# leopard-ai/betty

Hardware: AMD Instinct MI355X
Metric: hypergradient-steps/sec (CG K=20, 10M inner params) (higher is better)
Workload: dtype f32

## Files before the change

betty_amd/csrc/bhg_common.hpp:

```cpp
#pragma once
#include <hip/hip_runtime.h>
#include <stdint.h>
#include <stddef.h>
#include <stdio.h>
#include <string.h>

#include "bhg.h"

namespace bhg {

constexpr int kThreads = 256;
constexpr int kWaves = kThreads / 64;
constexpr int kChunk = BHG_CHUNK_ELEMS;
constexpr int kVecPerThread = kChunk / (kThreads * 4);
constexpr int kMaxBlocks = 1024;
constexpr int kInlineT = 32;
constexpr int kWriterT = 448;

constexpr size_t kWsScal = 0;
constexpr size_t kWsPartP = 128;
constexpr size_t kWsPartR = kWsPartP + 8 * kMaxBlocks;
constexpr size_t kWsBarrier = kWsPartR + 16 * kMaxBlocks;
constexpr size_t kWsTables = kWsBarrier + 256;
inline size_t ws_bytes(int T) {
  size_t b = kWsTables + 4 * sizeof(void*) * (size_t)(T > 0 ? T : 0);
  return (b + 255) & ~(size_t)255;
}

enum { S_RR_OLD = 0, S_PHP = 1, S_ALPHA = 2, S_RR_NEW = 3, S_BETA = 4, S_PP = 5 , S_ALPHA_RING = 10 ,
       S_NPART0 = 8  };

#define BHG_DBG_KEYS(X)                                                                                                      \
  X(mlp_wsk) X(mlp_wsk_maxk) X(mlp_wsk_depth) X(mlp_wsk_lds) X(wsl_depth) X(no_nt_slabs) X(gemm_no_xpose) X(mlp_no_fast)      \
  X(mlp_tn) X(split_target) X(split_cap) X(mlp_no_head) X(gram_ksplit) X(gram_kchunk) X(proj_graw_split) X(mlp_proj)         \
  X(mlp_hoist) X(hoist_wgs) X(proj_step_alone) X(mlp_no_side) X(mlp_no_fuse) X(mlp_no_outer_all) X(neumann_side)             \
  X(hoist_staged_mink) X(proj_alpha_alone) X(proj_small_alone) X(outer_order_by_work) X(outer_no_pre) X(outer_stagger)       \
  X(mlp_no_fused_solve) X(cg_eager_p) X(cg_x_every_iter) X(neumann_p_every_iter) X(head_no_prefetch) X(cg_spin_limit)        \
  X(packed_chain) X(packed_depth) X(packed_gram) X(proj_max_ratio) X(proj_ws_cap_mb) X(alpha_in_hoist) X(graw_v2) X(wskp_ragged) X(pstep_v2) X(pstep_unroll) X(rnew_in_graw) X(graw_cols) X(lin_first) X(lin_prio) X(lin_nub) X(lin_order) X(lin_update_next) X(lin_withhold_beta) X(neumann_vnew) X(cg_rhs_direct) X(packed_prepare) X(lin_deep) X(graw_kloop) X(lin_update_in_head) X(xcd_pairs) X(headu_head_first) X(fx_ksplit) X(head_j) X(head_j_tile)
enum DbgKey : int {
#define BHG_DBG_ENUM(n) DBG_##n,
  BHG_DBG_KEYS(BHG_DBG_ENUM)
#undef BHG_DBG_ENUM
  DBG_COUNT
};
constexpr int kDbgUnset = INT32_MIN;
#ifdef BHG_AB
extern int g_dbg[DBG_COUNT];
inline bool dbg_is_set(DbgKey k) { return g_dbg[k] != kDbgUnset; }
inline int dbg(DbgKey k, int dflt) { return g_dbg[k] == kDbgUnset ? dflt : g_dbg[k]; }
#else
constexpr bool dbg_is_set(DbgKey) { return false; }
constexpr int dbg(DbgKey, int dflt) { return dflt; }
#endif

constexpr int kStampKernels = 4, kStampBlocks = 4096, kStampSlots = 8;
#ifdef BHG_STAMPS
#ifdef __HIPCC__
#define BHG_STAMP(kid, slot)                                                                                            \
  do {                                                                                                                  \
    if (threadIdx.x == 0 && blockIdx.x < ::bhg::kStampBlocks) {                                                         \
      unsigned long long* sp_ = ::bhg::d_stamps;                                                                        \
      if (sp_) sp_[((kid) * ::bhg::kStampBlocks + blockIdx.x) * ::bhg::kStampSlots + (slot)] = wall_clock64();          \
    }                                                                                                                   \
  } while (0)
#endif
#else
#define BHG_STAMP(kid, slot) do { } while (0)
#endif

void set_error(const char* fmt, ...);
#define BHG_HIP_CHECK(expr)                                                        \
  do {                                                                             \
    hipError_t _e = (expr);                                                        \
    if (_e != hipSuccess) {                                                        \
      ::bhg::set_error("%s failed: %s (%s:%d)", #expr, hipGetErrorString(_e), __FILE__, \
                       __LINE__);                                                  \
      return BHG_ERR_HIP;                                                          \
    }                                                                              \
  } while (0)
#define BHG_REQUIRE(cond, msg)                                                     \
  do {                                                                             \
    if (!(cond)) {                                                                 \
      ::bhg::set_error("%s: %s", __func__, msg);                                   \
      return BHG_ERR_ARG;                                                          \
    }                                                                              \
  } while (0)

struct PtrTab {
  const void* const* dev;
  const void* inl[kInlineT];
};

int make_table(PtrTab* out, const void* const* host_ptrs, int T, void* ws, int slot,
               hipStream_t stream);

bool span_begin(int kind, hipEvent_t* a, hipEvent_t* b);

#ifdef __HIPCC__
__device__ __forceinline__ float* tab_ptr(const PtrTab& t, int i) {
  const void* p = t.dev ? t.dev[i] : t.inl[i];
  return (float*)p;
}

__device__ __forceinline__ float4 ld4(const float* __restrict__ base, int e, int len) {
  if (e + 4 <= len) return *reinterpret_cast<const float4*>(base + e);
  float4 r = make_float4(0.f, 0.f, 0.f, 0.f);
  if (e < len) r.x = base[e];
  if (e + 1 < len) r.y = base[e + 1];
  if (e + 2 < len) r.z = base[e + 2];
  return r;
}
__device__ __forceinline__ void st4(float* __restrict__ base, int e, int len, float4 v) {
  if (e + 4 <= len) {
    *reinterpret_cast<float4*>(base + e) = v;
    return;
  }
  if (e < len) base[e] = v.x;
  if (e + 1 < len) base[e + 1] = v.y;
  if (e + 2 < len) base[e + 2] = v.z;
}

// ... 142 lines not shown
```

betty_amd/csrc/bhg_mlp.hip:

```cpp
#include <stdlib.h>


#include "bhg_common.hpp"
#include "bhg_mlp_headj.hpp"

#ifdef BHG_STAMPS
namespace bhg { __device__ unsigned long long* d_stamps = nullptr; }
#endif

namespace bhg {
namespace {
#include "mlp/gemm.inc"

#include "mlp/outer.inc"

#include "mlp/scalars.inc"

#include "mlp/head.inc"

#include "mlp/wsk.inc"

#include "mlp/wskp.inc"

inline int wsk_mode(int chain_mode, int unfused_hint) {
  if (dbg_is_set(DBG_mlp_wsk)) return dbg(DBG_mlp_wsk, 0);
  if (chain_mode == FUSE_CG) return 2;
  if (chain_mode == FUSE_NEUMANN) return 3;
  return unfused_hint;
}
inline bool wsk_wanted(int mode, int pairs, int K) {
  if (mode == 1) return true;
  if (mode != 2 && mode != 3) return false;
  return pairs * K <= dbg(DBG_mlp_wsk_maxk, 1024);
}
inline int wsk_depth() {
  const int d = dbg(DBG_mlp_wsk_depth, 3);
  return d == 2 ? 2 : 3;
}
inline bool wsk_eligible(const WskArgs& a) {
  if (a.pairs < 1 || a.pairs > 2) return false;
  bool ok = a.M % 32 == 0 && a.N % 32 == 0 && a.K % 32 == 0 && a.K >= 32;
  for (int i = 0; i < a.pairs; ++i) ok = ok && (a.pr[i].lda & 3) == 0 && (a.pr[i].ldb & 3) == 0;
  return ok;
}
int64_t g_wsk_launches = 0;
int64_t g_hoist_launches = 0;
int64_t g_proj_iterations = 0;
int64_t g_lin_launches = 0;
template <int LB>
void launch_gemm_wsk(const WskArgs& a_in, hipStream_t st, bool staged = false) {
  WskArgs a = a_in;
  ++g_wsk_launches;
  a.ntm = a.M / 32;
  a.ntn = a.N / 32;
  bool bf = false;
  for (int i = 0; i < a.pairs; ++i) bf = bf || a.pr[i].mix != 0;
  const dim3 grid(a.ntm * a.ntn), block(64 * kWskWaves);
  const int d = wsk_depth();
  const bool force_staged = dbg(DBG_mlp_wsk_lds, 0) != 0;
  if ((staged || force_staged) && !bf) {
    const int lds = (int)(sizeof(float) * kWslWaveFloats * kWskWaves);
    static bool attr_done = false;
    if (!attr_done) {
      (void)hipFuncSetAttribute(reinterpret_cast<const void*>(k_gemm_wsk<LB, false, 2, true>), hipFuncAttributeMaxDynamicSharedMemorySize, lds);
      attr_done = true;
    }
#ifdef BHG_AB
    const int wsl_depth = dbg(DBG_wsl_depth, 2);
    if (wsl_depth == 3) {
      static bool attr3 = false;
      if (!attr3) {
        (void)hipFuncSetAttribute(reinterpret_cast<const void*>(k_gemm_wsk<LB, false, 3, true>), hipFuncAttributeMaxDynamicSharedMemorySize, lds);
        attr3 = true;
      }
      hipLaunchKernelGGL((k_gemm_wsk<LB, false, 3, true>), grid, block, lds, st, a);
      return;
    }
#endif
    hipLaunchKernelGGL((k_gemm_wsk<LB, false, 2, true>), grid, block, lds, st, a);
    return;
  }
#define BHG_WSK(BFV, DV) hipLaunchKernelGGL((k_gemm_wsk<LB, BFV, DV>), grid, block, 0, st, a)
  if (bf) {
    if (d == 2 || LB == LAYOUT_RC) BHG_WSK(true, 2); else BHG_WSK(true, LB == LAYOUT_RC ? 2 : 3);
  } else {
#ifdef BHG_AB
    if (d == 2) BHG_WSK(false, 2); else
// ... 428 lines not shown
  memset(w, 0, sizeof(*w));
  const bool head = use_head(m);
  int nrr = bias_blocks(m);
  for (int l = 0; l < m->L; ++l) nrr += outer_blocks(m, l, head);
  w->nRR = nrr;
  size_t off = 0;
  auto take = [&](size_t bytes) { void* p = base ? static_cast<char*>(base) + off : nullptr; off += (bytes + 255) & ~(size_t)255; return p; };
  w->partT1 = static_cast<double*>(take(sizeof(double) * m->Bp));
  w->partT2h = static_cast<double*>(take(sizeof(double) * m->Bp));
  w->partPP = static_cast<double*>(take(sizeof(double) * kMaxBlocks));
  w->partRR[0] = static_cast<double*>(take(sizeof(double) * 3 * nrr));
  w->partRR[1] = static_cast<double*>(take(sizeof(double) * 3 * nrr));
  int nt2 = 0;
  for (int l = 1; l + 1 < m->L; ++l) { w->t2_off[l] = nt2; nt2 += reduce_blocks(m->Bp * m->dims[l], m->dims[l]); }
  w->nT2 = nt2;
  HoistPlan hp;
  hoist_plan(m, &hp);
  const bool hj = headj_shape_ok(m, hp);
  w->nT2j = hj ? headj_tiles(m->Bp, m->dims[m->L - 1], 1) : 0;
  w->partT2 = static_cast<double*>(take(sizeof(double) * (nt2 + w->nT2j > 0 ? nt2 + w->nT2j : 1)));
  w->rz = static_cast<float*>(take(sizeof(float) * (size_t)m->Bp * m->dims[m->L]));
  w->rzx = static_cast<double*>(take(sizeof(double) * (size_t)m->Bp * m->dims[m->L]));
  w->hoist = static_cast<float*>(take(sizeof(float) * (hp.ok ? hp.floats : 1)));
  w->part_dot = static_cast<double*>(take(sizeof(double) * 2 * (hp.ok ? hp.dot_blocks : 1)));
  w->part_raw = static_cast<double*>(take(sizeof(double) * (hp.ok ? hp.raw_blocks : 1)));
  w->part_graw = static_cast<double*>(take(sizeof(double) * 3 * (hp.ok ? hp.graw_tiles : 1)));
  w->pscal = static_cast<double*>(take(sizeof(double) * 8));
  for (int i = 0; i < 2; ++i) w->pb0[i] = static_cast<float*>(take(sizeof(float) * (size_t)m->dims[1]));
  for (int i = 0; i < 2; ++i) w->pb1[i] = static_cast<float*>(take(sizeof(float) * (size_t)(m->L >= 2 ? m->dims[2] : 1)));
  w->gran = static_cast<unsigned long long*>(take(64 * 64));
  if (hp.ok) {
    const int L = m->L;
    const size_t Bp = (size_t)m->Bp;
    for (int l = 0; l + 1 < L; ++l) {
      w->hpk[l] = static_cast<float*>(take(sizeof(float) * Bp * m->dims[l]));
      if (l + 2 < L) w->Rhp[l] = static_cast<float*>(take(sizeof(float) * Bp * m->dims[l + 1]));
      if (l >= 1) {
        w->Wf[l] = static_cast<float*>(take(sizeof(float) * (size_t)m->dims[l + 1] * m->dims[l]));
        w->Wb[l] = static_cast<float*>(take(sizeof(float) * (size_t)m->dims[l + 1] * m->dims[l]));
        w->dpk[l] = static_cast<float*>(take(sizeof(float) * Bp * m->dims[l + 1]));
        w->Rdp[l] = static_cast<float*>(take(sizeof(float) * Bp * m->dims[l + 1]));
      }
    }
  }
  if (hj) {
    const size_t rj = (size_t)headj_rows(m->Bp, m->dims[m->L]);
    w->hj_J = static_cast<float*>(take(sizeof(float) * rj * m->dims[m->L - 2]));
    w->hj_Ap = static_cast<float*>(take(sizeof(float) * rj * m->dims[m->L - 1]));
  }
  w->bytes = off;
}

bool graw_single_on(bool packed, int Bp) { return packed && dbg(DBG_packed_gram, 1) != 0 && dbg(DBG_graw_v2, 1) != 0 && graw_batch_ok(Bp); }
bool rnew_keys_on() { return dbg(DBG_proj_small_alone, 0) == 0 && dbg(DBG_alpha_in_hoist, 1) != 0 && dbg(DBG_rnew_in_graw, 1) != 0; }

int pack_operands(const bhg_mlp* m, const FusedWs& w, hipStream_t st, bool weights_only = false) {
  PackArgs g{};
  int blk = 0;
  auto add = [&](const float* X, float* Xp, int R, int K, int kind) {
    if (g.n >= kPackMax) return false;
    g.p[g.n] = {X, Xp, R, K, kind};
    g.blk0[g.n] = blk;
    blk += pack_blocks(g.p[g.n]);
    ++g.n;
    return true;
  };
  const int L = m->L, Bp = m->Bp;
  bool ok = true;
  for (int l = 0; l + 1 < L && ok; ++l) {
    if (!weights_only || l == 0) ok = ok && add(m->h[l], w.hpk[l], Bp, m->dims[l], 0);
    if (l >= 1) {
      if (!weights_only) ok = ok && add(m->delta[l], w.dpk[l], Bp, m->dims[l + 1], 0);
      ok = ok && add(m->W[l], w.Wf[l], m->dims[l + 1], m->dims[l], 0);
      ok = ok && add(m->W[l], w.Wb[l], m->dims[l], m->dims[l + 1], 1);
    }
  }
  BHG_REQUIRE(ok, "too many layers for one packing launch");
  g.blk0[g.n] = blk;
  hipLaunchKernelGGL(k_pack, dim3(blk), dim3(256), 0, st, g);
  BHG_HIP_CHECK(hipGetLastError());
  return BHG_OK;
}

int build_head_j(const bhg_mlp* m, const FusedWs& w, hipStream_t st) {
  const int L = m->L, C = m->dims[L], K = m->dims[L - 1], N = m->dims[L - 2], RA = headj_rows(m->B, C);
  BHG_REQUIRE(w.nT2j > 0 && w.hj_J && w.hj_Ap && w.Wb[L - 2], "the head_j form was planned for a net it cannot take");
  if (int rc = launch_headj_pack(m->W[L - 1], m->mask[L - 2], w.hj_Ap, m->B, C, K, RA, st)) return rc;
  WskpBuilder wb;
  WskpProb q{};
  q.Ap = w.hj_Ap; q.Bq = w.Wb[L - 2]; q.RA = RA; q.RB = N; q.K = K; q.B = m->B * C; q.nsplit = 1;
  q.out = w.hj_J;
  wb.add(q);
  wb.launch(st);
  BHG_HIP_CHECK(hipGetLastError());
  return BHG_OK;
}

#include "mlp/solve_plan.inc"
#include "mlp/chain_plan.inc"

int hoist_products(const bhg_mlp* m, const void* const* dir, const ChainMode& cm, const ChainPlan& pl, hipStream_t st, ChainState* cs) {
  const int L = m->L, Bp = m->Bp, B = m->B;
  const HoistPlan* hp = pl.hp;
  float* hbase = pl.hoist;
  HoistArgs ha{};
  HoistRedArgs ra{};
  for (int i = 0; i < hp->n; ++i) {
    const int l = hp->layer[i];
    HoistProb& q = ha.p[i];
    q.A = hp->bwd[i] ? m->delta[l] : m->h[l];
    q.Bm = pl.cg ? ((cm.first && cm.rhs) ? static_cast<const float*>(cm.rhs[2 * l]) : cm.fa + cm.starts[2 * l]) : static_cast<const float*>(dir[2 * l]);
    q.slabs = hbase + hp->slab_off[i];
    q.K = hp->K[i]; q.N = hp->N[i]; q.splits = hp->splits[i]; q.rc = hp->bwd[i];
    q.lda = hp->K[i]; q.ldb = hp->bwd[i] ? hp->N[i] : hp->K[i];
    ha.blk0[i] = hp->blk0[i];
    HoistRedProb& rq = ra.p[i];
    rq.slabs = q.slabs; rq.G = hbase + hp->g_off[i]; rq.N = hp->N[i]; rq.splits = hp->splits[i];
    if (!hp->bwd[i] && l == 0) {
      rq.bias = static_cast<const float*>(dir[1]); rq.mask = m->mask[0]; rq.out = m->Rh[0];
      rq.outp = pl.packed ? cm.ws->Rhp[0] : nullptr;
    }
  }
  ha.blk0[hp->n] = hp->blk0[hp->n];
  ha.n = hp->n; ha.Bp = Bp; ha.gemm_blocks = hp->blk0[hp->n];
  const bool proj = pl.proj != 0;
  int rblk = 0;
  for (int i = 0; i < hp->n; ++i) { ra.blk0[i] = rblk; rblk += (Bp * (hp->N[i] / 4) + 255) / 256; }
  ra.blk0[hp->n] = rblk;
  if (!proj || cm.first) {
    ha.do_beta = (pl.cg && !cm.first && cm.beta && !proj) ? 1 : 0;
    ha.beta_blocks = ha.do_beta ? cm.beta_blocks : 0;
    if (ha.do_beta) ha.beta = *cm.beta;
    hipLaunchKernelGGL(k_hoist<FUSE_CG>, dim3(ha.gemm_blocks + (ha.do_beta ? cm.beta_blocks : 0)), dim3(256), 0, st, ha);
    ++g_hoist_launches;
    if (proj && pl.cg) for (int i = 0; i < hp->n; ++i) ra.p[i].G2 = hbase + hp->gr_off[i];
    ra.n = hp->n; ra.Bp = Bp; ra.B = B; ra.first = pl.cg ? cm.first : 1; ra.scal = cm.scal;
    hipLaunchKernelGGL(k_hoist_reduce, dim3(rblk), dim3(256), 0, st, ra);
  } else if (pl.vnew) {
    ++g_proj_iterations;
  } else {
    ProjArgs pa{};
    for (int i = 0; i < hp->n; ++i) {
      ProjProb& q = pa.p[i];
      q.Gr = hbase + (pl.cg ? hp->gr_off[i] : hp->g_off[i]); q.Gp = hbase + hp->g_off[i]; q.Graw = hbase + hp->graw_off[i]; q.N = hp->N[i];
      if (!pl.graw_single && graw_split() && !(hp->bwd[i] == 0 && hp->layer[i] == 0)) q.Graw2 = q.Graw + (size_t)Bp * hp->N[i];
      if (pl.rnew) q.Graw = nullptr;
      if (!hp->bwd[i] && hp->layer[i] == 0) {
        q.bias = static_cast<const float*>(dir[1]); q.mask = m->mask[0]; q.out = m->Rh[0];
        q.outp = pl.packed ? cm.ws->Rhp[0] : nullptr;
      }
      pa.blk0[i] = ra.blk0[i];
    }
    pa.blk0[hp->n] = rblk;
    pa.n = hp->n; pa.Bp = Bp; pa.B = B; pa.kpar_prev = cm.kpar ^ 1; pa.shift = cm.shift; pa.scal = pl.cg ? cm.scal : nullptr; pa.alpha = cm.alpha;
    if (pl.cg && pl.proj >= 2 && proj_step_merged()) {
      ProjStepArgs g{};
      g.pa = pa;
      ProjScalArgs& sa = g.sa;
      sa.part_dot = cm.ws->part_dot; sa.dot_blocks = hp->dot_blocks;
      sa.part_raw = cm.ws->part_raw; sa.raw_blocks = graw_blocks(hp, Bp);
      if (pl.graw_single) {
        const int gt = graw_tile_count(hp, Bp);
        sa.part_dot = cm.ws->part_graw; sa.dot_blocks = gt;
        sa.part_raw = cm.ws->part_graw + 2 * (size_t)gt; sa.raw_blocks = gt;
      }
      sa.part = cm.beta->part; sa.part_stride = cm.ws->nRR;
      sa.off0 = pl.part_base_w[L - 1]; sa.n0 = outer_blocks(m, L - 1, pl.head); sa.off1 = pl.part_base_bias; sa.n1 = bias_blocks(m);
      sa.r_small = cm.beta->r; sa.p_small = cm.beta->p; sa.snt = cm.beta->nt;
      int small_total = 0;
// ... 45 lines not shown
        }
        for (int t = 0; t < sa.snt; ++t) { ps.t.slen[t] = sa.slen[t]; ps.t.soff[t] = sa.soff[t]; }
        if (pl.lin) { cs->lin_ps = ps; cs->lin_nu = (h.nub > 0 ? h.nub : rblk) + sgrid; cs->lin_U = U; }
#ifdef BHG_AB
        else if (U == 2) hipLaunchKernelGGL(k_pstep<2>, dim3(rblk + sgrid), dim3(256), 0, st, ps);
        else if (U == 1) hipLaunchKernelGGL(k_pstep<1>, dim3(rblk + sgrid), dim3(256), 0, st, ps);
#endif
        else hipLaunchKernelGGL(k_pstep<4>, dim3(rblk + sgrid), dim3(256), 0, st, ps);
      } else {
#ifdef BHG_AB
        hipLaunchKernelGGL(k_proj_step, dim3(rblk + sgrid), dim3(256), 0, st, g);
#else
        BHG_REQUIRE(false, "internal: every plan of the product takes k_pstep (<= 16 small tensors, the packed closing launch)");
#endif
      }
    } else {
      hipLaunchKernelGGL(k_proj_update, dim3(rblk), dim3(256), 0, st, pa);
    }
    ++g_proj_iterations;
  }
  return BHG_OK;
}

int lin_first_product(const bhg_mlp* m, const void* const* dir, const ChainMode& cm, const ChainPlan& pl, hipStream_t st, ChainState* cs) {
  const int L = m->L, Bp = m->Bp, B = m->B, K = m->dims[1], N = m->dims[2];
  const HoistPlan* hp = pl.hp;
  float* hbase = pl.hoist;
  const float* c = static_cast<const float*>(dir[3]);
  const float* Gf = hbase + hp->g_off[hp->gf[1]];
  BHG_REQUIRE(cm.first || cs->lin_nu > 0, "no update blocks for the linear first product");
  WskplArgs la{};
  WskpProb& q = la.a;
  q.Ap = cm.first ? cm.ws->Rhp[0] : hbase + hp->rh0rp_off;
  q.Bq = cm.ws->Wf[1]; q.RA = Bp; q.RB = N; q.K = K; q.B = B; q.nsplit = 1;
  q.mask = m->mask[1]; q.out = m->Rh[1]; q.outp = cm.ws->Rhp[1];
  q.znew = hbase + hp->z1_off[cm.kpar];
  if (cm.first) { q.addend = Gf; q.bias = c; }
  else {
    q.addend = hbase + hp->gr_off[hp->gf[1]]; q.addend2 = pl.gp1(cm.kpar ^ 1);
    q.bias = cm.fa + cm.starts[3]; q.bias2 = cs->lin_ps.h.p1_rd;
    q.zold = hbase + hp->z1_off[cm.kpar ^ 1];
    q.gran = cm.ws->gran;
  }
  const int rider_blocks = pl.gram_in_chain ? (Bp / 32) * (Bp / 32) : 0;
  wskp_tiling(&q, false);
  int na = (q.nfull * (q.RB / 32) + q.nstrip + 7) & ~7;
  if (dbg(DBG_wskp_ragged, 1) == 2 || (dbg(DBG_wskp_ragged, 1) == 1 && na + rider_blocks > chip_cus()) ||
      (!cm.first && cs->lin_ps.h.nub > 0)) {
    wskp_tiling(&q, true);
    na = (q.nfull * (q.RB / 32) + q.nstrip + 7) & ~7;
  }
  la.na = na;
  if (pl.gram_in_chain) {
    float* tnew = hbase + hp->tslab_off[1] + (size_t)cm.kpar * Bp * Bp;
    float* tnewp = pl.graw2 ? hbase + hp->tslabp_off[1] + (size_t)cm.kpar * Bp * Bp : nullptr;
    la.r0 = {cm.ws->hpk[1], q.Ap, tnew, tnewp, K, 0};
    la.r0_old = cm.first ? nullptr : hbase + hp->tslab_off[1] + (size_t)(cm.kpar ^ 1) * Bp * Bp;
  }
  la.nu = cm.first ? 0 : cs->lin_nu;
  const bool upd_next = !cm.first && L == 4 && dbg(DBG_lin_update_next, 1) != 0 && cs->lin_ps.h.nub == 0;
  if (upd_next) {
    la.ns = cs->lin_nu - cs->lin_ps.h.update_blocks;
    la.nt = na + rider_blocks;
  } else if (!cm.first && L > 4 && cs->lin_ps.h.nub == 0) {
    la.ns = cs->lin_nu - cs->lin_ps.h.update_blocks;
    la.nt = na + rider_blocks;
    la.upd_first = 1;
  } else
  if (!cm.first && dbg(DBG_lin_order, 0) != 0) {
    la.ns = cs->lin_nu - (cs->lin_ps.h.nub > 0 ? cs->lin_ps.h.nub : cs->lin_ps.h.update_blocks);
    la.nt = na + rider_blocks;
  }
  la.ps = cs->lin_ps;
  BHG_REQUIRE(cm.first || la.ns > 0 || cs->lin_ps.h.update_blocks <= 2 * chip_cus(),
              "update blocks ahead of the publisher would not all be resident: use the default order");
  const int grid = (upd_next ? la.ns : la.nu) + na + rider_blocks;
  cs->lin_update_pending = upd_next;
  BHG_REQUIRE(cm.first || cs->lin_U == 4, "the update blocks inside k_wskpl are built for four float4 per thread");
#ifdef BHG_AB
  if (la.ps.h.nub > 0) hipLaunchKernelGGL((k_wskpl<2, 4, true>), dim3(grid), dim3(64 * kWskpWaves), 0, st, la); else
#endif
  hipLaunchKernelGGL((k_wskpl<2, 4, false>), dim3(grid), dim3(64 * kWskpWaves), 0, st, la);
  ++g_lin_launches;
  if (cm.first)
    BHG_HIP_CHECK(hipMemcpyAsync(hbase + hp->rb0c_off, cm.fa + cm.starts[1], sizeof(float) * (size_t)m->dims[1],
                                 hipMemcpyDeviceToDevice, st));
  return BHG_OK;
}

int hoist_forward(const bhg_mlp* m, const void* const* dir, const ChainMode& cm, const ChainPlan& pl, hipStream_t st, int staged_mink,
                  ChainState* cs) {
  const int L = m->L, Bp = m->Bp, B = m->B;
  const HoistPlan* hp = pl.hp;
  float* hbase = pl.hoist;
  for (int l = 1; l + 1 < L; ++l) {
    const int K = m->dims[l], N = m->dims[l + 1];
    const float* c = static_cast<const float*>(dir[2 * l + 1]);
    const float* Gf = hbase + hp->g_off[hp->gf[l]];
    if (pl.packed) {
    if (pl.lin && l == 1) {
      if (int rc = lin_first_product(m, dir, cm, pl, st, cs)) return rc;
    } else {
      WskpBuilder wb;
      WskpProb q{};
      q.Ap = cm.ws->Rhp[l - 1]; q.Bq = cm.ws->Wf[l]; q.RA = Bp; q.RB = N; q.K = K; q.B = B; q.nsplit = 1;
      if (l == L - 2) {
        const int riders = (pl.gram_in_chain && l == 1) ? (Bp / 32) * (Bp / 32) : 0;
        const int tiles_l = (Bp / 32) * (N / 32);
        int sp = (chip_cus() - riders) / tiles_l;
        const int cap = pick_splits((N + pl.tn - 1) / pl.tn, K, 1);
        if (sp > cap) sp = cap;
        if (sp > K / 64) sp = K / 64;
        if (sp < 1) sp = 1;
        if (pl.head_j && cs->lin_update_pending) {
          cs->head_fuse = {nullptr, 0, Bp * N, c, m->mask[l], m->Rh[l], hbase + hp->gr_off[hp->gf[l]]};
          cs->fuse_head = true;
          cs->head_j = true;
          continue;
        }
        q.nsplit = sp; q.raw = 1; q.out = m->partial;
        cs->head_fuse = {m->partial, sp, Bp * N, c, m->mask[l], m->Rh[l], (pl.lin_head && !cm.first) ? hbase + hp->gr_off[hp->gf[l]] : Gf};
        cs->fuse_head = true;
      } else {
        q.bias = c; q.mask = m->mask[l]; q.addend = Gf; q.out = m->Rh[l]; q.outp = cm.ws->Rhp[l];
      }
      wb.add(q);
      if (pl.gram_in_chain && l == 1) {
        WskpProb t{};
        t.Ap = cm.ws->hpk[l]; t.Bq = cm.ws->Rhp[l - 1]; t.RA = Bp; t.RB = Bp; t.K = K; t.B = B;
        t.nsplit = 1; t.raw = 1; t.out = hbase + hp->tslab_off[l]; t.outp = pl.graw2 ? hbase + hp->tslabp_off[l] : nullptr;
        wb.add(t);
      }
      if (cs->lin_update_pending && wb.g.n == 1 && !pl.lin_head) {
        launch_wskpu(wb.g.p[0], cs->lin_ps, cs->lin_ps.h.update_blocks, st);
        cs->lin_update_pending = false;
      } else wb.launch(st);
    }
      if (pl.gram_in_chain && cm.first && l == 1) {
        WskpBuilder sb;
        for (int j = 0; j + 1 < L; ++j) {
          WskpProb u{};
          u.Ap = cm.ws->hpk[j]; u.Bq = cm.ws->hpk[j]; u.RA = Bp; u.RB = Bp; u.K = m->dims[j]; u.B = B; u.raw = 1;
          u.nsplit = 1;
          u.out = hbase + hp->s_off[j]; u.outp = hbase + hp->sp_off[j];
          if (!sb.add(u)) { sb.launch(st); sb.add(u); }
          if (j >= 1) {
            u.Ap = cm.ws->dpk[j]; u.Bq = cm.ws->dpk[j]; u.K = m->dims[j + 1]; u.out = hbase + hp->d_off[j]; u.outp = hbase + hp->dp_off[j];
            if (!sb.add(u)) { sb.launch(st); sb.add(u); }
          }
        }
        sb.launch(st);
        cs->sd_in_chain = true;
      }
      continue;
    }
    if (l == L - 2) {
      GemmArgs a{};
      a.pr[0] = {m->Rh[l - 1], m->W[l], K, K};
      a.pairs = 1; a.M = Bp; a.N = N; a.K = K;
      a.splits = pick_splits((N + pl.tn - 1) / pl.tn, K, 1);
      a.out = m->partial; a.ldo = N; a.out_rows = Bp;
      launch_gemm<LAYOUT_KC, LAYOUT_KC>(a, pl.tn, st);
      cs->head_fuse = {m->partial, a.splits, Bp * N, c, m->mask[l], m->Rh[l], Gf};
      cs->fuse_head = true;
    } else {
      WskArgs w{};
      w.pr[0] = {m->Rh[l - 1], m->W[l], K, K}; w.pairs = 1; w.M = Bp; w.N = N; w.K = K; w.B = B;
      w.bias = c; w.mask = m->mask[l]; w.out = m->Rh[l]; w.addend = Gf;
      launch_gemm_wsk<LAYOUT_KC>(w, st, K >= staged_mink);
    }
  }
  BHG_REQUIRE(!cs->lin_update_pending || pl.lin_head, "the update blocks found no launch to ride in");
  return BHG_OK;
}

int hoist_head(const bhg_mlp* m, const void* const* dir, const ChainMode& cm, const ChainPlan& pl, hipStream_t st, ChainState* cs) {
  const int L = m->L, Bp = m->Bp, B = m->B;
  if (cs->lin_update_pending && cs->head_j) {
    const int l = L - 1, K = m->dims[l], N = m->dims[l + 1];
    BHG_REQUIRE(cs->fuse_head && pl.cg && pl.packed && cm.ws->nT2j > 0 && !cm.rzx_acc, "k_headj was planned for a head it cannot run");
    HeadjLaunch a{};
    a.h = m->h[l]; a.W = m->W[l]; a.V = static_cast<const float*>(dir[2 * l]); a.cb = static_cast<const float*>(dir[2 * l + 1]);
    a.prob = m->prob; a.sd = m->sd; a.rd = m->Rd[l];
    a.K = K; a.C = N; a.B = B; a.rows = Bp;
    a.delta_top = (const float*)m->delta[l]; a.mask_prev = (const float*)m->mask[l - 1]; a.rd_prev = m->Rd[l - 1]; a.rd_prev_p = cm.ws->Rdp[l - 1];
    a.partT1 = cm.ws->partT1; a.rz_out = cm.ws->rz;
    a.bias2 = cs->head_fuse.bias; a.mask2 = cs->head_fuse.mask; a.addend = cs->head_fuse.addend;
    a.addend2 = pl.gp2(cm.kpar ^ 1); a.gran = cm.ws->gran;
    a.J = cm.ws->hj_J; a.Rh1 = m->Rh[l - 2]; a.K1 = m->dims[l - 1];
    a.Rh1p = cm.ws->Rhp[l - 2]; a.W2p = cm.ws->Wf[l - 1]; a.rh_out = m->Rh[l - 1];
    a.tile_shape = dbg(DBG_head_j_tile, kHeadjTile);
    const int nt = headj_tiles(Bp, K, a.tile_shape);
    if (nt <= B) { a.partT2 = cm.ws->partT2h; a.t2n = B; cs->head_j_nt = 0; }
    else { a.partT2 = cm.ws->partT2 + cm.ws->nT2; a.t2n = nt; cs->head_j_nt = nt; }
    a.ps = &cs->lin_ps; a.ps_bytes = sizeof(cs->lin_ps); a.nu = cs->lin_ps.h.update_blocks;
    if (int rc = launch_headj(a, st)) return rc;
    cs->lin_update_pending = false;
  } else if (cs->lin_update_pending) {
    const int l = L - 1, K = m->dims[l], N = m->dims[l + 1];
    BHG_REQUIRE(cs->fuse_head && pl.cg && pl.packed && N <= 12 && K <= 512, "k_headu was planned for a head it cannot run");
    HeaduArgs ha{};
    ha.Rh = (const float*)m->Rh[l - 1]; ha.h = m->h[l]; ha.W = m->W[l]; ha.V = static_cast<const float*>(dir[2 * l]);
    ha.cb = static_cast<const float*>(dir[2 * l + 1]); ha.prob = m->prob; ha.sd = m->sd; ha.rd = m->Rd[l];
    ha.K = K; ha.C = N; ha.B = B; ha.mode = HEAD_JVP;
    ha.delta_top = (const float*)m->delta[l]; ha.mask_prev = (const float*)m->mask[l - 1]; ha.rd_prev = m->Rd[l - 1];
    ha.fz = cs->head_fuse;
    ha.partT1 = cm.ws->partT1; ha.partT2h = cm.ws->partT2h; ha.rz_out = cm.ws->rz; ha.rzx_acc = cm.rzx_acc; ha.rzx_first = cm.first;
    ha.rows = Bp; ha.rd_prev_p = cm.ws->Rdp[l - 1];
    ha.addend2 = pl.gp2(cm.kpar ^ 1); ha.gran = cm.ws->gran;
    ha.nu = cs->lin_ps.h.update_blocks; ha.ps = cs->lin_ps; ha.head_first = dbg(DBG_headu_head_first, 1);
    hipLaunchKernelGGL(k_headu<4>, dim3(ha.nu + Bp), dim3(256), (size_t)K * sizeof(float), st, ha);
    cs->lin_update_pending = false;
  } else {
    const int l = L - 1, K = m->dims[l], N = m->dims[l + 1];
    launch_head_forward(st, Bp, (const float*)m->Rh[l - 1], m->h[l], m->W[l], static_cast<const float*>(dir[2 * l]),
                        static_cast<const float*>(dir[2 * l + 1]), m->prob, m->sd, m->Rd[l], K, N, B, HEAD_JVP, nullptr, nullptr,
                        (const float*)m->delta[l], (const float*)m->mask[l - 1], m->Rd[l - 1], &cs->head_fuse,
                        pl.cg ? cm.ws->partT1 : nullptr, pl.cg ? cm.ws->partT2h : nullptr, pl.cg ? cm.ws->rz : nullptr, cm.rzx_acc, cm.first,
                        pl.packed ? cm.ws->Rdp[l - 1] : nullptr);
  }
  return BHG_OK;
}

void hoist_backward(const bhg_mlp* m, const ChainMode& cm, const ChainPlan& pl, hipStream_t st, int staged_mink) {
  const int L = m->L, Bp = m->Bp, B = m->B;
  const HoistPlan* hp = pl.hp;
  float* hbase = pl.hoist;
  for (int l = L - 2; l >= 1; --l) {
    const int K = m->dims[l + 1], N = m->dims[l];
    if (pl.packed) {
      WskpBuilder wb;
      WskpProb q{};
      q.Ap = cm.ws->Rdp[l]; q.Bq = cm.ws->Wb[l]; q.RA = Bp; q.RB = N; q.K = K; q.B = B; q.nsplit = 1;
// ... 1277 lines not shown
```

Measured before the change: 776.0.

## Build head J in one fused kernel riding the Gram launch

Adds a dedicated J-build kernel that multiplies W3 by the mask on the fly inside an MFMA loop, replacing the separate pack step plus generic product. By default the J tiles and the rb0c copy are appended as extra blocks to the existing Gram (sd) launch, which removes two or three small launches and a device-to-device memcpy per hypergradient step. In exchange the fused kernel needs more LDS and registers, and the extra blocks may contend with the Gram blocks.

```diff
diff --git a/betty_amd/csrc/bhg_common.hpp b/betty_amd/csrc/bhg_common.hpp
--- a/betty_amd/csrc/bhg_common.hpp
+++ b/betty_amd/csrc/bhg_common.hpp
@@ -36,7 +36,7 @@
   X(mlp_hoist) X(hoist_wgs) X(proj_step_alone) X(mlp_no_side) X(mlp_no_fuse) X(mlp_no_outer_all) X(neumann_side)             \
   X(hoist_staged_mink) X(proj_alpha_alone) X(proj_small_alone) X(outer_order_by_work) X(outer_no_pre) X(outer_stagger)       \
   X(mlp_no_fused_solve) X(cg_eager_p) X(cg_x_every_iter) X(neumann_p_every_iter) X(head_no_prefetch) X(cg_spin_limit)        \
-  X(packed_chain) X(packed_depth) X(packed_gram) X(proj_max_ratio) X(proj_ws_cap_mb) X(alpha_in_hoist) X(graw_v2) X(wskp_ragged) X(pstep_v2) X(pstep_unroll) X(rnew_in_graw) X(graw_cols) X(lin_first) X(lin_prio) X(lin_nub) X(lin_order) X(lin_update_next) X(lin_withhold_beta) X(neumann_vnew) X(cg_rhs_direct) X(packed_prepare) X(lin_deep) X(graw_kloop) X(lin_update_in_head) X(xcd_pairs) X(headu_head_first) X(fx_ksplit) X(head_j) X(head_j_tile)
+  X(packed_chain) X(packed_depth) X(packed_gram) X(proj_max_ratio) X(proj_ws_cap_mb) X(alpha_in_hoist) X(graw_v2) X(wskp_ragged) X(pstep_v2) X(pstep_unroll) X(rnew_in_graw) X(graw_cols) X(lin_first) X(lin_prio) X(lin_nub) X(lin_order) X(lin_update_next) X(lin_withhold_beta) X(neumann_vnew) X(cg_rhs_direct) X(packed_prepare) X(lin_deep) X(graw_kloop) X(lin_update_in_head) X(xcd_pairs) X(headu_head_first) X(fx_ksplit) X(head_j) X(head_j_tile) X(head_j_build)
 enum DbgKey : int {
 #define BHG_DBG_ENUM(n) DBG_##n,
   BHG_DBG_KEYS(BHG_DBG_ENUM)
diff --git a/betty_amd/csrc/bhg_mlp.hip b/betty_amd/csrc/bhg_mlp.hip
--- a/betty_amd/csrc/bhg_mlp.hip
+++ b/betty_amd/csrc/bhg_mlp.hip
@@ -3,6 +3,7 @@
 
 #include "bhg_common.hpp"
 #include "bhg_mlp_headj.hpp"
+#include "bhg_mlp_jbuild.hpp"
 
 #ifdef BHG_STAMPS
 namespace bhg { __device__ unsigned long long* d_stamps = nullptr; }
@@ -597,9 +598,18 @@
   return BHG_OK;
 }
 
+JbuildLaunch head_j_operands(const bhg_mlp* m, const FusedWs& w) {
+  const int L = m->L, C = m->dims[L];
+  return JbuildLaunch{m->W[L - 1], m->mask[L - 2], w.Wb[L - 2], w.hj_J, m->B, C, m->dims[L - 1], m->dims[L - 2], headj_rows(m->B, C)};
+}
+bool head_j_rides(const bhg_mlp* m) {
+  return dbg(DBG_head_j_build, kHeadJBuild) == 2 && dbg(DBG_packed_gram, 1) != 0 && dbg(DBG_packed_depth, 2) == 2 && 2 * m->L - 3 <= kWskpMax;
+}
 int build_head_j(const bhg_mlp* m, const FusedWs& w, hipStream_t st) {
   const int L = m->L, C = m->dims[L], K = m->dims[L - 1], N = m->dims[L - 2], RA = headj_rows(m->B, C);
   BHG_REQUIRE(w.nT2j > 0 && w.hj_J && w.hj_Ap && w.Wb[L - 2], "the head_j form was planned for a net it cannot take");
+  if (head_j_rides(m)) return BHG_OK;
+  if (dbg(DBG_head_j_build, kHeadJBuild) != 0) return launch_jbuild(head_j_operands(m, w), st);
   if (int rc = launch_headj_pack(m->W[L - 1], m->mask[L - 2], w.hj_Ap, m->B, C, K, RA, st)) return rc;
   WskpBuilder wb;
   WskpProb q{};
@@ -811,7 +821,7 @@
 #endif
   hipLaunchKernelGGL((k_wskpl<2, 4, false>), dim3(grid), dim3(64 * kWskpWaves), 0, st, la);
   ++g_lin_launches;
-  if (cm.first)
+  if (cm.first && !(pl.head_j && pl.gram_in_chain && head_j_rides(m)))
     BHG_HIP_CHECK(hipMemcpyAsync(hbase + hp->rb0c_off, cm.fa + cm.starts[1], sizeof(float) * (size_t)m->dims[1],
                                  hipMemcpyDeviceToDevice, st));
   return BHG_OK;
@@ -878,6 +888,13 @@
             if (!sb.add(u)) { sb.launch(st); sb.add(u); }
           }
         }
+        if (pl.head_j && head_j_rides(m)) {
+          BHG_REQUIRE(pl.lin && sb.g.n == 2 * L - 3 && cm.ws->nT2j > 0 && cm.ws->hj_J, "the J tiles found no Gram launch to ride in");
+          sb.tile(false);
+          sb.g.blk0[sb.g.n] = sb.blk;
+          if (int rc = launch_sdj(&sb.g, sizeof(sb.g), sb.blk, head_j_operands(m, *cm.ws), cm.fa + cm.starts[1], hbase + hp->rb0c_off,
+                                  m->dims[1], st)) return rc;
+        } else
         sb.launch(st);
         cs->sd_in_chain = true;
       }
diff --git a/betty_amd/csrc/bhg_mlp_jbuild.hip b/betty_amd/csrc/bhg_mlp_jbuild.hip
--- /dev/null
+++ b/betty_amd/csrc/bhg_mlp_jbuild.hip
@@ -0,0 +1,232 @@
+#include <stdlib.h>
+
+#include "bhg_mlp_jbuild.hpp"
+
+#ifdef BHG_STAMPS
+#undef BHG_STAMP
+#define BHG_STAMP(kid, slot) do { } while (0)
+#endif
+
+namespace bhg {
+namespace {
+#include "mlp/gemm.inc"
+#include "mlp/outer.inc"
+#include "mlp/scalars.inc"
+#include "mlp/head.inc"
+#include "mlp/wsk.inc"
+#include "mlp/wskp.inc"
+
+struct JbArgs {
+  const float* W3; const float* mask2; const float* W2p; float* J;
+  int BC, C, K, N, RA;
+};
+
+constexpr int kJbRblk = 2;
+constexpr int kJbRows = 16 * kJbRblk;
+constexpr int jb_lds(int cblk) { return kWskpWaves * 32 * (16 * cblk + 1); }
+
+template <int RBLK, int CBLK>
+__device__ __forceinline__ void jb_loop(const float* const (&pw)[RBLK], const float* const (&pm)[RBLK], const bool (&ok)[RBLK],
+                                        const float* __restrict__ gB, const int64_t sB, const int nch, f32x4 (&acc)[RBLK][CBLK]) {
+  constexpr int D = 2;
+  f32x4 aw[D][RBLK][2], am[D][RBLK][2];
+  f32x4 sb[D][CBLK][2];
+  auto load = [&](const int d, int ch) {
+    ch = min(ch, nch - 1);
+#pragma unroll
+    for (int h = 0; h < 2; ++h) {
+      const float* pb = gB + (int64_t)(2 * ch + h) * sB;
+#pragma unroll
+      for (int rb = 0; rb < RBLK; ++rb) {
+        aw[d][rb][h] = *reinterpret_cast<const f32x4*>(pw[rb] + 16 * (2 * ch + h));
+        am[d][rb][h] = *reinterpret_cast<const f32x4*>(pm[rb] + 16 * (2 * ch + h));
+      }
+#pragma unroll
+      for (int cb = 0; cb < CBLK; ++cb) sb[d][cb][h] = *reinterpret_cast<const f32x4*>(pb + cb * 256);
+    }
+  };
+  auto compute = [&](const int d) {
+#pragma unroll
+    for (int h = 0; h < 2; ++h) {
+      f32x4 a[RBLK];
+#pragma unroll
+      for (int rb = 0; rb < RBLK; ++rb)
+#pragma unroll
+        for (int j = 0; j < 4; ++j) a[rb][j] = ok[rb] ? aw[d][rb][h][j] * am[d][rb][h][j] : 0.f;
+#pragma unroll
+      for (int c = 0; c < 4; ++c) {
+#pragma unroll
+        for (int rb = 0; rb < RBLK; ++rb)
+#pragma unroll
+          for (int cb = 0; cb < CBLK; ++cb)
+            acc[rb][cb] = __builtin_amdgcn_mfma_f32_16x16x4f32(a[rb][c], sb[d][cb][h][c], acc[rb][cb], 0, 0, 0);
+      }
+    }
+  };
+#pragma unroll
+  for (int d = 0; d < D; ++d) {
+    load(d, d);
+    __builtin_amdgcn_sched_barrier(0);
+  }
+  int s = 0;
+  for (; s + 2 * D <= nch; s += D) {
+#pragma unroll
+    for (int d = 0; d < D; ++d) {
+      compute(d);
+      __builtin_amdgcn_sched_barrier(0);
+      load(d, s + D + d);
+      __builtin_amdgcn_sched_barrier(0);
+    }
+  }
+#pragma unroll
+  for (int d = 0; d < D; ++d) {
+    if (s + d < nch) compute(d);
+    if (s + D + d < nch) load(d, s + D + d);
+  }
+  s += D;
+#pragma unroll
+  for (int d = 0; d < D; ++d)
+    if (s + d < nch) compute(d);
+}
+
+template <int RBLK, int CBLK>
+__device__ __forceinline__ void jb_tile(const JbArgs& g, const int t, float* __restrict__ sPf) {
+  constexpr int TR = 16 * RBLK, TC = 16 * CBLK, TCP = TC + 1;
+  static_assert(RBLK % 2 == 0 && (32 * TC) % (64 * kWskpWaves) == 0, "the meeting goes 32 rows at a time, whole outputs per thread");
+  const int RA = g.RA, N = g.N, K = g.K, C = g.C;
+  const int ntm = (RA + TR - 1) / TR, ntn = N / TC;
+  int tm = t % ntm, tn = t / ntm;
+  if ((ntn & 7) == 0) { const int j = t >> 3; tm = j % ntm; tn = (j / ntm) * 8 + (t & 7); }
+  const int m0 = TR * tm, n0 = TC * tn;
+  const int lane = threadIdx.x & 63;
+  const int wave = __builtin_amdgcn_readfirstlane(threadIdx.x >> 6);
+  const int li = lane & 15, lk = lane >> 4;
+  const int nct = K / 32;
+  const int c0 = (int)(((int64_t)wave * nct) / kWskpWaves), c1 = (int)(((int64_t)(wave + 1) * nct) / kWskpWaves);
+  const int nch_w = c1 - c0;
+  f32x4 acc[RBLK][CBLK];
+#pragma unroll
+  for (int a = 0; a < RBLK; ++a)
+#pragma unroll
+    for (int b = 0; b < CBLK; ++b)
+#pragma unroll
+      for (int r = 0; r < 4; ++r) acc[a][b][r] = 0.f;
+  if (nch_w > 0) {
+    const float* pw[RBLK]; const float* pm[RBLK]; bool ok[RBLK];
+#pragma unroll
+    for (int rb = 0; rb < RBLK; ++rb) {
+      const int r = m0 + 16 * rb + li;
+      ok[rb] = r < g.BC;
+      const int rr = ok[rb] ? r : 0;
+      const int b = rr / C, c = rr - b * C;
+      pw[rb] = g.W3 + (int64_t)c * K + 32 * c0 + 4 * lk;
+      pm[rb] = g.mask2 + (int64_t)b * K + 32 * c0 + 4 * lk;
+    }
+    const int64_t sB = (int64_t)16 * N;
+    const float* gB = g.W2p + (int64_t)(2 * c0) * sB + (n0 + li) * 16 + 4 * lk;
+    jb_loop<RBLK, CBLK>(pw, pm, ok, gB, sB, nch_w, acc);
+  }
+  float* sW = sPf + wave * (32 * TCP);
+  constexpr int kOutPer = 32 * TC / (64 * kWskpWaves);
+#pragma unroll
+  for (int half = 0; half < RBLK / 2; ++half) {
+    if (half > 0) __syncthreads();
+#pragma unroll
+    for (int rb = 0; rb < 2; ++rb)
+#pragma unroll
+      for (int cbk = 0; cbk < CBLK; ++cbk)
+#pragma unroll
+        for (int r = 0; r < 4; ++r) sW[(16 * rb + 4 * lk + r) * TCP + 16 * cbk + li] = acc[2 * half + rb][cbk][r];
+    __syncthreads();
+#pragma unroll
+    for (int u = 0; u < kOutPer; ++u) {
+      const int e = threadIdx.x + 64 * kWskpWaves * u;
+      const int row = e / TC, col = e % TC;
+      const int m = m0 + 32 * half + row;
+      float v = 0.f;
+#pragma unroll
+      for (int w = 0; w < kWskpWaves; ++w) v += sPf[w * (32 * TCP) + row * TCP + col];
+      if (m < RA) g.J[(int64_t)m * N + n0 + col] = m < g.BC ? v : 0.f;
+    }
+  }
+}
+
+template <int CBLK>
+__global__ __launch_bounds__(64 * kWskpWaves) void k_jbuild(JbArgs g) {
+  __shared__ float sPf[jb_lds(CBLK)];
+  jb_tile<kJbRblk, CBLK>(g, (int)blockIdx.x, sPf);
+}
+
+struct SdjArgs {
+  WskpArgs g;
+  JbArgs j;
+  int nsd, nj;
+  const float* cp_src; float* cp_dst; int cp_n;
+};
+static_assert(sizeof(SdjArgs) <= 3900, "kernel arguments of k_sdj must fit the kernarg segment");
+
+template <int CBLK>
+__global__ __launch_bounds__(64 * kWskpWaves) void k_sdj(SdjArgs a) {
+  constexpr int kLds = jb_lds(CBLK) > kWskpLds ? jb_lds(CBLK) : kWskpLds;
+  __shared__ float sPf[kLds];
+  __shared__ double red[kWskpWaves];
+  const int blk = (int)blockIdx.x;
+  if (blk < a.nsd) {
+    int i = 0;
+    while (i + 1 < a.g.n && blk >= a.g.blk0[i + 1]) ++i;
+    const WskpProb q = a.g.p[i];
+    wskp_body<2>(q, blk - a.g.blk0[i], sPf, red, a.g);
+    return;
+  }
+  if (blk < a.nsd + a.nj) { jb_tile<kJbRblk, CBLK>(a.j, blk - a.nsd, sPf); return; }
+  for (int i = threadIdx.x; i < a.cp_n; i += 64 * kWskpWaves) a.cp_dst[i] = a.cp_src[i];
+}
+
+inline int jb_cblk(int N) { return N % 96 == 0 ? 6 : (N % 64 == 0 ? 4 : 2); }
+
+int jb_args(const JbuildLaunch& a, JbArgs* g) {
+  BHG_REQUIRE(a.W3 && a.mask2 && a.W2p && a.J, "NULL argument");
+  BHG_REQUIRE(a.B >= 1 && a.C >= 1 && a.K >= 32 && a.K % 32 == 0 && a.N >= 32 && a.N % 32 == 0 && a.RA % 32 == 0 && a.RA >= a.B * a.C,
+              "the J build was planned for a shape it cannot take");
+  BHG_REQUIRE((((uintptr_t)a.W3 | (uintptr_t)a.mask2 | (uintptr_t)a.W2p) & 15) == 0, "operands must be 16-byte aligned");
+  *g = JbArgs{a.W3, a.mask2, a.W2p, a.J, a.B * a.C, a.C, a.K, a.N, a.RA};
+  return BHG_OK;
+}
+}
+
+int jbuild_tiles(int RA, int N) { return ((RA + kJbRows - 1) / kJbRows) * (N / (16 * jb_cblk(N))); }
+
+int launch_jbuild(const JbuildLaunch& a, hipStream_t st) {
+  JbArgs g;
+  if (int rc = jb_args(a, &g)) return rc;
+  const dim3 grid(jbuild_tiles(a.RA, a.N)), block(64 * kWskpWaves);
+  switch (jb_cblk(a.N)) {
+    case 6: hipLaunchKernelGGL(k_jbuild<6>, grid, block, 0, st, g); break;
+    case 4: hipLaunchKernelGGL(k_jbuild<4>, grid, block, 0, st, g); break;
+    default: hipLaunchKernelGGL(k_jbuild<2>, grid, block, 0, st, g); break;
+  }
+  BHG_HIP_CHECK(hipGetLastError());
+  return BHG_OK;
+}
+
+int launch_sdj(const void* sd, size_t sd_bytes, int nsd, const JbuildLaunch& a, const float* cp_src, float* cp_dst, int cp_n, hipStream_t st) {
+  BHG_REQUIRE(sd && sd_bytes == sizeof(WskpArgs), "the Gram launch's arguments do not match this build");
+  BHG_REQUIRE(cp_src && cp_dst && cp_n >= 0, "NULL argument");
+  SdjArgs s{};
+  memcpy(&s.g, sd, sizeof(WskpArgs));
+  BHG_REQUIRE(s.g.n >= 1 && s.g.n <= kWskpMax && nsd > 0 && nsd % 8 == 0 && s.g.blk0[0] == 0 && s.g.blk0[s.g.n] == nsd,
+              "the Gram launch's block table does not match its grid");
+  if (int rc = jb_args(a, &s.j)) return rc;
+  s.nsd = nsd; s.nj = jbuild_tiles(a.RA, a.N);
+  s.cp_src = cp_src; s.cp_dst = cp_dst; s.cp_n = cp_n;
+  const dim3 grid(nsd + s.nj + 1), block(64 * kWskpWaves);
+  switch (jb_cblk(a.N)) {
+    case 6: hipLaunchKernelGGL(k_sdj<6>, grid, block, 0, st, s); break;
+    case 4: hipLaunchKernelGGL(k_sdj<4>, grid, block, 0, st, s); break;
+    default: hipLaunchKernelGGL(k_sdj<2>, grid, block, 0, st, s); break;
+  }
+  BHG_HIP_CHECK(hipGetLastError());
+  return BHG_OK;
+}
+
+}
diff --git a/betty_amd/csrc/bhg_mlp_jbuild.hpp b/betty_amd/csrc/bhg_mlp_jbuild.hpp
--- /dev/null
+++ b/betty_amd/csrc/bhg_mlp_jbuild.hpp
@@ -0,0 +1,21 @@
+#pragma once
+#include <stddef.h>
+
+#include "bhg_common.hpp"
+
+namespace bhg {
+
+struct JbuildLaunch {
+  const float* W3;
+  const float* mask2;
+  const float* W2p;
+  float* J;
+  int B, C, K, N, RA;
+};
+constexpr int kHeadJBuild = 2;
+int jbuild_tiles(int RA, int N);
+int launch_jbuild(const JbuildLaunch& a, hipStream_t st);
+
+int launch_sdj(const void* sd, size_t sd_bytes, int nsd, const JbuildLaunch& a, const float* cp_src, float* cp_dst, int cp_n, hipStream_t st);
+
+}
```

Result: no change. 782.9, median of 6 (+0.9%).
